# Infinidat/slimfastq

Hardware: AMD Instinct MI355X
Metric: MB/s FASTQ compressed (higher is better)
Workload: dtype u8/u32 integer; 1 GPU; synthetic 10M x 150 bp Illumina reads per GPU, full qlts+gens+recs, frozen tables (one chain per lane), -l 3; level=3, block_reads=1024, prior_step=-1, blocks_per_gpu=9766, tables=frozen, chains_per_gpu=253906, raw_bytes_per_gpu=3702038404, parallelism=1 GPU

## Files before the change

slimfastq_amd/csrc/api.cpp:

```cpp
#include <hip/hip_runtime.h>

#include <algorithm>
#include <cmath>
#include <cstdarg>
#include <cstdlib>
#include <cstdio>
#include <cstring>
#include <string>
#include <vector>
#include <chrono>
#include <functional>
#include <future>
#include <thread>
#include <atomic>
#include <mutex>
#include <condition_variable>

#include "kernels.h"

namespace {

struct HostTimes {
    bool on; std::chrono::steady_clock::time_point t0; std::vector<std::pair<const char*, double>> marks;
    HostTimes() : on(getenv("SFQ_HOST_TIMING") != nullptr), t0(std::chrono::steady_clock::now()) {}
// ... 51 lines not shown
    EE_HEAD_END,
    EE_M0_BEGIN, EE_M0_END, EE_M1_BEGIN, EE_M1_END, EE_M2_BEGIN, EE_M2_END, EE_M3_BEGIN, EE_M3_END,
    EE_PACK_BEGIN, EE_PACK_END,
    EE_FRAME_K_BEGIN,
    EE_TEXT_FORK,
    EE_QLT_CODE_BEGIN, EE_QLT_CODE_END,
    EE_GEN_CODE_BEGIN, EE_GEN_CODE_END,
    EE_REC_CODE_BEGIN,
    EE_NEVER_READ,
    EE_QLT_LIST_HOME,
    EE_QLT_ROWS_BUILT,
    EE_LINES_INDEXED,
    EE_FRAME_K_END,
    EE_REC_FREQS_HOME,
    EE_REC_CODE_END,
    EE_COUNT
};
enum {
    ED_BEGIN,
    ED_HEAD_END,
    ED_FORK,
    ED_QLT_END,
    ED_GEN_END,
    ED_REC_END,
    ED_END,
    ED_GEN_BEGIN,
    ED_OVER_FORK,
    ED_OVER_LINES_END,
    ED_LISTS_COPIED,
    ED_COUNT
// ... 9 lines not shown
    bool rec_copy_pending = false;
    bool rec_blob_pending = false;
    std::string err;
    u64 table_budget = 0;
    u64 dev_total = 0;
    u32 wave_slots = 8192;
    u32 epoch_base = 0;
    Tables tab;
    DevBuf chunk_base, scan_tmp, line_off, status, blocks, arena, blk_stream_off, stream_total,
           lens, blob_off, blob, in_stage, out_stage;
    DevBuf slen, qlen, pfg, pfq, soff, qoff, seq_stage, qual_stage, hdr_stage, hlen, hoff, hso, hsc, rsize, roff, d_first;
    DevBuf hist, rows66, ptmp, prior_w, prior_wovf, prior_ls, prior_lh, tickets;
    DevBuf gm_T, gm_slen, gm_boff, gm_soff, gm_scan, gm_stage, gm_tok, gm_csz, gm_idx;
    DevBuf qrows, qdec, qesc, qw, csz, coff, gcnt, grows, glog, gcost, gbins, gfill, hcnt, hfreq, rrows, rdec, rmap, rflags, rtok, excf, cflags;
    DevBuf chn_len, chn_off, chn_out;
    DevBuf pslot, plist;
    DevBuf segn, segoff, segrec;
    DevBuf oflags, okbytes, ofpos, okoff, ofilt, orecmap, olist, line_off_o, ono, opiece, otxt[3], osize_all, oroff_all, oroff_k, ocnt;
    u32 r_hot = 0, r_hot_dec = 0;
    bool blobs_from_encode = false;
    bool unsettled = false;
    bool counts_only = false; u32 sample_scale = 1;
    struct { const u8* ptr = nullptr; u64 nbytes = 0, nrec = 0, print = 0; bool marks = false, valid = false; } framed;
    struct { bool valid = false, rec = false; u32 q_rows = 0; } counts;
    void* pin = nullptr; size_t pin_cap = 0;
    void* pin2 = nullptr; size_t pin2_cap = 0;
    std::vector<u8> chain_blob;
    std::vector<u8> rec_prior_blob;
    std::vector<u8> chain_tmp;
    bool prior_on = false;
// ... 549 lines not shown
    const u32 ngen = gp.ngen = gen_bounds(nblocks, gp.bound);
    if (ngen < 3) return SFQ_OK;
    const u32* bound = gp.bound;
    int rc;
    gp.tb = gm_table_bits(ca.nbytes);
    const u64 br = ca.block_reads;
    gp.r2 = std::min<u64>(nrec, (u64)bound[2] * br);
    gp.cap = std::min<u64>(ca.nbytes, gp.r2 * ((u64)max_line + 1));
    if ((rc = reserve(ctx, ctx->gm_T, (size_t)8 << gp.tb))) return rc;
    if ((rc = reserve(ctx, ctx->gm_slen, (size_t)gp.r2 * 4 + 64))) return rc;
    if ((rc = reserve(ctx, ctx->gm_boff, ((size_t)gp.r2 + 1) * 8))) return rc;
    if ((rc = reserve(ctx, ctx->gm_soff, ((size_t)gp.r2 + 1) * 8))) return rc;
    if ((rc = reserve(ctx, ctx->gm_scan, ((size_t)nrec / 1024 + 4) * 8 + 65536))) return rc;
    if ((rc = reserve(ctx, ctx->gm_stage, (size_t)gp.cap + 64))) return rc;
    if ((rc = reserve(ctx, ctx->gcost, 64))) return rc;
    HIPC(hipMemsetAsync(ctx->gm_T.p, 0xFF, (size_t)8 << gp.tb, st));
    HIPC(hipMemsetAsync(ctx->gcost.p, 0, 64, st));
    if ((rc = gm_stage_upto(ctx, ca, gp.r2, 0, st))) return rc;
    gp.cg = ca;
    gp.cg.st_buf = (const u8*)ctx->gm_stage.p; gp.cg.st_bytes = gp.cap; gp.cg.st_off = (const u64*)ctx->gm_soff.p; gp.cg.st_len = (const u32*)ctx->gm_slen.p;
    auto recs = [&](u32 b0, u32 b1) { return (u64)(b1 - b0) * br; };
    launch_gm_insert(gp.cg, bound[0], bound[1], recs(bound[0], bound[1]), max_line, (u64*)ctx->gm_T.p, gp.tb, st);
    u16 costs[8];
    for (u32 lv = 0; lv < 4; lv++) {
        const u32 fo = lv == 0 ? 64u : lv == 1 ? 40u : lv == 2 ? 24u : 16u;
        costs[lv] = (u16)(12 * 1024 - log2fp_u32(4096u - 3u * fo)); costs[4 + lv] = (u16)(12 * 1024 - log2fp_u32(fo));
    }
    const u64 r1 = (u64)bound[1] * br;
    launch_gm_price(gp.cg, r1, gp.r2, (u64)gen_count_stride(recs(bound[1], bound[2])) * GEN_PRE, max_line, r1, (const u8*)ctx->gm_stage.p, gp.cap, (const u64*)ctx->gm_soff.p,
                    (const u32*)ctx->gm_slen.p, (const u64*)ctx->gm_T.p, gp.tb, costs, (u64*)ctx->gcost.p, st);
    HIPC(hipMemcpyAsync((u8*)ctx->pin + PIN_GEN_OFF, ctx->gcost.p, 16, hipMemcpyDeviceToHost, st));
    return SFQ_OK;
}
// ... 124 lines not shown
    ctx->table_budget = tot / 10 * 7;
    *out = ctx;
    return SFQ_OK;
}

void sfq_ctx_destroy(sfq_ctx* ctx) {
    if (!ctx) return;
    (void)hipSetDevice(ctx->dev);
    (void)hipStreamSynchronize(ctx->st);
    DevBuf* all[] = { &ctx->tab.q_slots, &ctx->tab.q_hdr, &ctx->tab.p_slots, &ctx->tab.p_hdr, &ctx->tab.g_tab,
        &ctx->chunk_base, &ctx->scan_tmp, &ctx->line_off, &ctx->status, &ctx->blocks, &ctx->arena,
        &ctx->blk_stream_off, &ctx->stream_total, &ctx->lens, &ctx->blob_off, &ctx->blob, &ctx->in_stage, &ctx->out_stage,
        &ctx->slen, &ctx->qlen, &ctx->pfg, &ctx->pfq, &ctx->soff, &ctx->qoff, &ctx->seq_stage, &ctx->qual_stage,
        &ctx->hdr_stage, &ctx->hlen, &ctx->hoff, &ctx->hso, &ctx->hsc, &ctx->rsize, &ctx->roff, &ctx->d_first,
        &ctx->hist, &ctx->rows66, &ctx->prior_w, &ctx->prior_wovf, &ctx->prior_ls, &ctx->prior_lh, &ctx->tickets,
        &ctx->hcnt, &ctx->hfreq, &ctx->rrows, &ctx->rdec, &ctx->rmap, &ctx->rflags, &ctx->rtok, &ctx->ptmp, &ctx->qrows, &ctx->qdec, &ctx->qesc, &ctx->qw, &ctx->csz, &ctx->coff, &ctx->gcnt, &ctx->grows, &ctx->glog, &ctx->gcost, &ctx->gbins, &ctx->gfill, &ctx->gm_T, &ctx->gm_slen, &ctx->gm_boff, &ctx->gm_soff, &ctx->gm_scan, &ctx->gm_stage, &ctx->gm_tok, &ctx->gm_csz, &ctx->gm_idx, &ctx->excf, &ctx->cflags, &ctx->segn, &ctx->segoff, &ctx->segrec, &ctx->pslot, &ctx->plist, &ctx->chn_len, &ctx->chn_off, &ctx->chn_out,
        &ctx->oflags, &ctx->okbytes, &ctx->ofpos, &ctx->okoff, &ctx->ofilt, &ctx->orecmap, &ctx->olist, &ctx->line_off_o, &ctx->ono, &ctx->opiece,
        &ctx->otxt[0], &ctx->otxt[1], &ctx->otxt[2], &ctx->osize_all, &ctx->oroff_all, &ctx->oroff_k, &ctx->ocnt,
        &ctx->crc_tab, &ctx->crc_tiles, &ctx->crc_grps, &ctx->crc_bounds, &ctx->crc_out, &ctx->stats_acc, &ctx->qmap_dev,
        &ctx->pair_work, &ctx->pair_in, &ctx->pair_out, &ctx->pick_out, &ctx->sel_out, &ctx->trim_out, &ctx->ovl_out, &ctx->mrg_out, &ctx->dd_out, &ctx->scr_out };
    for (DevBuf* b : all) release(*b);
    (void)sfq_dedup_set_destroy(ctx);
    (void)sfq_screen_set_destroy(ctx);
    if (ctx->pin) (void)hipHostFree(ctx->pin);
    if (ctx->pin2) (void)hipHostFree(ctx->pin2);
    if (ctx->crc_pin) (void)hipHostFree(ctx->crc_pin);
    for (auto& e : ctx->crc_ev) if (e) (void)hipEventDestroy(e);
    if (ctx->st_crc) (void)hipStreamDestroy(ctx->st_crc);
    if (ctx->stats_pin) (void)hipHostFree(ctx->stats_pin);
    if (ctx->qmap_pin) (void)hipHostFree(ctx->qmap_pin);
    if (ctx->pair_pin) (void)hipHostFree(ctx->pair_pin);
// ... 196 lines not shown
    const u32 block_reads = p.block_reads ? p.block_reads : (u32)std::min<u64>(nrec, 0xFFFFFFFFu);
    const u64 nblocks64 = (nrec + block_reads - 1) / block_reads;
    if (nblocks64 > (1u << 24)) return fail(ctx, SFQ_E_ARG, "too many blocks (%llu)", (unsigned long long)nblocks64);
    const u32 nblocks = (u32)nblocks64;
    const bool frozen = p.tables == SFQ_TABLES_FROZEN && p.block_reads != 0 && p.kernel == 0;
    int g_bits = p.gen_bits ? p.gen_bits : level_gen_bits(p.level);
    if (!p.gen_bits && p.block_reads) {
        const double bases = (frozen ? (double)nrec : (double)block_reads) * ((double)nbytes / (double)nrec) * 0.5;
        int cap = 12;
        while (cap < 26 && (double)(1u << cap) < bases) cap += 2;
        g_bits = std::min(g_bits, cap);
    }
    if (g_bits < 2 || g_bits > 26 ) return fail(ctx, SFQ_E_ARG, "gen_bits %d out of range", g_bits);
    if ((rc = reserve(ctx, ctx->blocks, (size_t)nblocks * sizeof(BlockDesc)))) return rc;
    launch_block_prepare(d_fastq, (const u64*)ctx->line_off.p, nrec, block_reads, (BlockDesc*)ctx->blocks.p, nblocks, nbytes, p.level, g_bits, st);
    const bool crc_pass = ctx->crc_on && !priors_only;
    if (crc_pass) {
        if ((rc = crc_reserve(ctx, d_fastq_in, 0, nbytes_in, nblocks))) return rc;
        HIPC(hipEventRecord(ctx->crc_ev[CRC_EV_FORK], st));
        HIPC(hipStreamWaitEvent(ctx->st_crc, ctx->crc_ev[CRC_EV_FORK], 0));
        launch_crc_block_bounds((const u64*)ctx->line_off.p, 4ull * block_reads, nblocks, nbytes_in, (u64*)ctx->crc_bounds.p, ctx->st_crc);
        if ((rc = crc_queue(ctx, d_fastq_in, nbytes_in, nblocks, ctx->st_crc))) return rc;
        HIPC(hipEventRecord(ctx->crc_ev[CRC_EV_DONE], ctx->st_crc));
    }
    const bool stats_pass = ctx->stats_on && !priors_only;
    if (stats_pass) {
        if ((rc = stats_ready(ctx))) return rc;
        HIPC(hipEventRecord(ctx->stats_ev[0], st));
        HIPC(hipStreamWaitEvent(ctx->st_stats, ctx->stats_ev[0], 0));
        HIPC(hipMemsetAsync(ctx->stats_acc.p, 0, (size_t)text_stats_acc_bytes(), ctx->st_stats));
// ... 17 lines not shown
            return fail(ctx, SFQ_E_ARG, "SFQ_PRIOR_COUNTS: no counts installed (sfq_set_prior_counts / sfq_count_priors come first; any other encode drops them)");
        if (ctx->counts.q_rows != q_rows) return fail(ctx, SFQ_E_ARG, "SFQ_PRIOR_COUNTS: the counts were installed for %u quality contexts, level %d has %u", ctx->counts.q_rows, p.level, q_rows);
        if (need_rec && !ctx->counts.rec) return fail(ctx, SFQ_E_ARG, "SFQ_PRIOR_COUNTS: the installed counts hold no header sample (they were counted for adaptive tables), frozen tables need one");
    }
    if (given && ctx->prior_blob.empty()) return fail(ctx, SFQ_E_ARG, "SFQ_PRIOR_GIVEN: no quality prior installed (sfq_set_qlt_prior)");
    if (given && frozen && (models & SFQ_M_REC) && ctx->rec_prior_blob.empty()) return fail(ctx, SFQ_E_ARG, "SFQ_PRIOR_GIVEN: no header prior installed (sfq_set_rec_prior)");
    if (!given) { ctx->prior_blob.clear(); ctx->rec_prior_blob.clear(); }
    ctx->rec_blob_pending = false; ctx->rec_copy_pending = false;
    ctx->chain_blob.clear();
    if (frozen && !prior_step) prior_step = SFQ_PRIOR_AUTO;
    u32 slots = 0;
    const u32 KR = 2;
    const u32 nblocks_r = (nblocks + KR - 1) / KR * KR;
    ModelArgs a;
    u32* tickets = nullptr;
    auto setup_tables = [&]() -> int {
        int rc;
        if ((rc = ensure_tables(ctx, nblocks_r, q_rows, (u32)g_bits, frozen ? (models & ~(SFQ_M_QLT | SFQ_M_GEN)) : models, &slots))) return rc;
        if (p.kernel == 0) {
            if (slots < KR) return fail(ctx, SFQ_E_NOMEM, "table budget %llu B holds %u block slot(s); the kernels need %u", (unsigned long long)ctx->table_budget, slots, KR);
            slots &= ~(KR - 1);
        }
        if ((rc = advance_epoch(ctx, nblocks))) return rc;
        fill_model_args(ctx, a, nblocks, p.level, (u32)g_bits, p.block_reads != 0);
        a.fq = d_fastq;
        a.rec_map = n_over ? (const u32*)ctx->orecmap.p : nullptr;
        if ((rc = reserve(ctx, ctx->tickets, 64))) return rc;
        HIPC(hipMemsetAsync(ctx->tickets.p, 0, 64, st));
        tickets = (u32*)ctx->tickets.p;
        return SFQ_OK;
    };
    const u32 order[4] = { SFQ_M_QLT, frozen ? SFQ_M_REC : SFQ_M_GEN, SFQ_M_USR, frozen ? SFQ_M_GEN : SFQ_M_REC };
    const int tslot[4] = { SFQ_T_QLT, frozen ? SFQ_T_REC : SFQ_T_GEN, SFQ_T_USR, frozen ? SFQ_T_GEN : SFQ_T_REC };
    hipStream_t mst[4] = { st, ctx->st_aux[0], ctx->st_aux[1], ctx->st_aux[2] };
    if (prior_step == SFQ_PRIOR_AUTO || (ctx->counts_only && prior_step == 0)) {
        const u64 per_rec = std::min<u64>(std::max<u64>(1, nbytes / nrec / 2), PRIOR_SYMBOLS);
        prior_step = (u32)std::min<u64>(std::max<u64>(1, nrec * per_rec / 24000000ull), 0x7FFFFFFFull);
        if (nbytes / nrec <= 4000) prior_step = (u32)std::max<u64>(prior_step, (nrec + 131071) / 131072);
    }
    if (ctx->counts_only && prior_step && prior_step < SFQ_PRIOR_COUNTS)
        prior_step = (u32)std::min<u64>((u64)prior_step * std::max<u32>(1u, ctx->sample_scale), 0x7FFFFFFFull);
    bool hist_launched = false;
    if (frozen && !given && !counted && prior_step && (models & SFQ_M_QLT)) {
// ... 9 lines not shown
    else HIPC(hipStreamSynchronize(st));
    const u32 h_status = h_status2[0], max_hdr = h_status2[1], max_line = h_status2[2], min_hdr = ~h_status2[4];
    if (h_status == (u32)(-SFQ_E_FORMAT)) return fail(ctx, SFQ_E_FORMAT, "fastq file: expecting '@' / '+' line prefixes (usrs.cpp:162-167)");
    if (h_status) return fail(ctx, -(int)h_status, "record over the line limits: headers up to 8190 bytes; base and quality lines up to 65534 in format 6 (-B 0; the reference would write oversize side streams, usrs.cpp:269-301, which this library does not), up to 1 Gi in the block format; or an empty base line");

    ChainArgs ca;
    memset(&ca, 0, sizeof ca);
    u32 nchains = 0, nsub = 0;
    GenPlan gplan; GmPlan gmplan;
    ChainGeoArgs ggeo; memset(&ggeo, 0, sizeof ggeo);
    const u32* gen_csz = nullptr;
    const bool flat_quads_req = getenv("SFQ_FLAT_QUADS") != nullptr;
    const bool gm = frozen && !exc_classic;
    u32 seg_len = 0;
    std::vector<u32> seg_blk;
    if (frozen) {
        u32 cr = p.chain_reads ? p.chain_reads : (u32)default_chain_reads(nrec, nbytes);
        if (p.chain_reads & SFQ_CHAIN_SEGMENT_FLAG) { seg_len = p.chain_reads & ~SFQ_CHAIN_SEGMENT_FLAG; cr = 1; if (!seg_len) return fail(ctx, SFQ_E_ARG, "SFQ_CHAIN_SEGMENT(0)"); }
        else if (!p.chain_reads && cr == 1 && nrec < 204800) {
            const u64 segs_want = SFQ_CHAINS_WANT - 8192 - std::min<u64>(nrec / 2, 100000);
            const u64 want = std::min<u64>(std::max<u64>(4096, nbytes / 2 / segs_want), 1u << 20);
            if (max_line > want) seg_len = (u32)want;
        }
        if (!p.chain_reads && !seg_len)
            while (cr < block_reads && (u64)nblocks * ((block_reads + cr - 1) / cr) > SFQ_CHAINS_WANT) cr++;
        ca.geo.chain_reads = (u32)std::min<u64>(std::min(cr, block_reads), nrec);
        ca.geo.cpb = (block_reads + ca.geo.chain_reads - 1) / ca.geo.chain_reads;
        if (!p.chain_reads) ca.geo.chain_reads = std::max<u32>(1u, (u32)((std::min<u64>(block_reads, nrec) + ca.geo.cpb - 1) / ca.geo.cpb));
        const u32 last_nrec = (u32)(nrec - (u64)(nblocks - 1) * block_reads);
        const u64 nc = (u64)(nblocks - 1) * ca.geo.cpb + (last_nrec + ca.geo.chain_reads - 1) / ca.geo.chain_reads;
// ... 15 lines not shown
            for (u32 b = 0; b < nblocks; b++) seg_blk[b] = (u32)(h_off[std::min<u64>((u64)(b + 1) * block_reads, nrec)] - h_off[(u64)b * block_reads]);
            if ((rc = reserve(ctx, ctx->segrec, (size_t)nchains * 4 + 16))) return rc;
            launch_seg_fill((const u64*)ctx->segoff.p, nrec, (u32*)ctx->segrec.p, st);
            ca.seg_len = seg_len; ca.seg_off = (const u64*)ctx->segoff.p; ca.seg_rec = (const u32*)ctx->segrec.p;
        }
        {
            const u32 cpb_want = std::max<u32>(1u, 61440u / nblocks);
            const u32 rfloor = nbytes / nrec > 4000 ? 16u : 128u;
            const u32 rcr0 = std::max<u32>(rfloor, (block_reads + cpb_want - 1) / cpb_want);
            const u32 rcr = (u32)std::min<u64>(std::min<u32>(std::max<u32>(rcr0, ca.geo.chain_reads), block_reads), nrec);
            ca.rgeo.chain_reads = rcr;
            ca.rgeo.cpb = (block_reads + rcr - 1) / rcr;
            nsub = ca.rgeo.nchains = (u32)((u64)(nblocks - 1) * ca.rgeo.cpb + (last_nrec + rcr - 1) / rcr);
        }
        if ((rc = reserve(ctx, ctx->csz, ((size_t)nchains * 2 + (size_t)nsub * 2) * 4))) return rc;
        HIPC(hipMemsetAsync(ctx->csz.p, 0, ((size_t)nchains * 2 + (size_t)nsub * 2) * 4, st));
        ggeo = ca.geo;
        if (gm && !seg_len) {
            const u64 per_rec = std::max<u64>(1, nbytes / std::max<u64>(1, nrec));
            const u64 gwant = std::max<u64>((GM_CHAIN_FLOOR + per_rec - 1) / per_rec, (nrec + GM_CHAIN_WANT - 1) / GM_CHAIN_WANT);
            const u32 gfloor = (u32)std::min<u64>(gwant, ca.geo.chain_reads);
            ggeo.cpb = (block_reads + gfloor - 1) / gfloor;
            ggeo.chain_reads = std::max<u32>(1u, (u32)((std::min<u64>(block_reads, nrec) + ggeo.cpb - 1) / ggeo.cpb));
            ggeo.cpb = (block_reads + ggeo.chain_reads - 1) / ggeo.chain_reads;
            const u64 ngc = (u64)(nblocks - 1) * ggeo.cpb + (last_nrec + ggeo.chain_reads - 1) / ggeo.chain_reads;
            if (ngc > 0x7FFFFFFFull || ggeo.chain_reads >= ca.geo.chain_reads) ggeo = ca.geo;
            else {
                ggeo.nchains = (u32)ngc;
                if ((rc = reserve(ctx, ctx->gm_csz, (size_t)ggeo.nchains * 4))) return rc;
                HIPC(hipMemsetAsync(ctx->gm_csz.p, 0, (size_t)ggeo.nchains * 4, st));
            }
        }
        if ((rc = reserve_pinned(ctx, PIN_BYTES + (size_t)q_rows * 66 * 4))) return rc;
        if ((rc = setup_tables())) return rc;
        HIPC(hipEventRecord(ctx->ev[EE_TEXT_FORK], st));
        if (!priors_only) {
            for (int m = 1; m < 4; m++) { HIPC(hipStreamWaitEvent(mst[m], ctx->ev[EE_TEXT_FORK], 0)); HIPC(hipEventRecord(ev_model_begin(ctx, m), mst[m])); }
            a.batch0 = 0; a.nbatch = std::min(slots, nblocks_r);
            ca.m = a;
            if (models & SFQ_M_REC) { if ((rc = rec_prior_begin(ctx, a, nrec, given, counted, mst[1], max_hdr))) return rc; }
            if (models & SFQ_M_GEN) {
                if (gm) { if ((rc = gm_begin(ctx, ca, nblocks, nrec, max_line, mst[3], gmplan))) return rc; }
                else if ((rc = gen_tables_begin(ctx, ca, nblocks, (u32)g_bits, max_line, mst[3], gplan))) return rc;
            }
        } else if (models & SFQ_M_REC) {
            HIPC(hipStreamWaitEvent(mst[1], ctx->ev[EE_TEXT_FORK], 0));
            if ((rc = rec_prior_begin(ctx, a, nrec, given, counted, mst[1], max_hdr))) return rc;
        }
    }
    u32* h_rows66 = nullptr;
    if (given && (models & SFQ_M_QLT)) {
        if ((rc = ensure_prior_buffers(ctx, q_rows))) return rc;
        if (!hist_cleared) HIPC(hipMemsetAsync(ctx->hist.p, 0, (size_t)q_rows * 64 * 4, st));
        if ((rc = upload_prior(ctx, q_rows, st, !frozen))) return rc;
        HIPC(hipEventRecord(ctx->ev[EE_HEAD_END], st));
        ctx->prior_on = true;
    } else if (prior_step && (models & SFQ_M_QLT)) {
        if ((rc = ensure_prior_buffers(ctx, q_rows))) return rc;
// ... 35 lines not shown
            launch_qlt_frozen_rows((const u32*)ctx->rows66.p, q_rows, (u32*)ctx->qrows.p, nullptr, st);
            ca.qrows = (const u32*)ctx->qrows.p; ca.qesc = (const u32*)ctx->qesc.p;
            ca.q_hot = 0; ca.q_rows = q_rows;
            const u32 want_hot = (p.lds_rows == SFQ_LDS_ROWS_NONE || given || !prior_step) ? 0u : p.lds_rows ? std::min<u32>(p.lds_rows, 1024u)
                                 : nchains >= 150000u ? 800u : 0u;
            if (want_hot) {
                const size_t img_bytes = (size_t)q_rows / 4 + (size_t)want_hot * 100 + 64;
                if ((rc = reserve(ctx, ctx->qw, img_bytes + (size_t)q_rows * 4 + 256))) return rc;
                u8* img = (u8*)ctx->qw.p; u32* info = (u32*)(img + ((img_bytes + 15) & ~(size_t)15)); u32* ctot = info + 16;
                launch_hot_rows((const u32*)ctx->hist.p, (const u32*)ctx->rows66.p, (const u32*)ctx->qrows.p, q_rows, want_hot, ctot, img, info, st);
                ca.q_hot = want_hot; ca.qh_img = img; ca.qh_info = info;
            }
            HIPC(hipEventRecord(ctx->ev[EE_HEAD_END], st));
        }
    }
    if (!frozen) { if ((rc = setup_tables())) return rc; }
    if (priors_only) {
        if (ctx->prior_on && !given) {
            if ((rc = qlt_prior_blob_now(ctx, h_rows66, q_rows, st))) return rc;
        }
        if (frozen && (models & SFQ_M_REC)) { if ((rc = rec_prior_finish(ctx, given, mst[1]))) return rc; if ((rc = rec_prior_copy_back(ctx, mst[1]))) return rc; if ((rc = rec_prior_blob_now(ctx))) return rc; }
        HIPC(hipStreamSynchronize(mst[1]));
        HIPC(hipStreamSynchronize(st));
        ctx->prior_on = false;
        res->n_records = nrec; res->n_blocks = nblocks;
        return SFQ_OK;
    }
    u32 gen_on = 0;
    const bool exc_rice = frozen && !exc_classic;
    if (frozen) {
        a.batch0 = 0; a.nbatch = std::min(slots, nblocks_r);
// ... 80 lines not shown
                }
            }
        }
        if (order[m] == SFQ_M_USR && n_over) {
            const u64 ooff[3] = { arena_main, arena_main + over_cap, arena_main + 2 * over_cap };
            const u32 ocap[3] = { (u32)over_cap, (u32)over_cap, (u32)over_cap };
            launch_over_encode_w(a, d_file, (const u64*)ctx->line_off_o.p, (const u32*)ctx->olist.p, n_over, ooff, ocap, mst[m]);
        }
        HIPC(hipEventRecord(ev_model_end(ctx, m), mst[m]));
        if (m) HIPC(hipStreamWaitEvent(st, ev_model_end(ctx, m), 0));
    }
    }
    ht.mark("chains queued");
    HIPC(hipEventRecord(ctx->ev[EE_PACK_BEGIN], st));

    if ((rc = reserve(ctx, ctx->blk_stream_off, (size_t)nblocks * SFQ_NSTREAMS * 8))) return rc;
    if ((rc = reserve(ctx, ctx->stream_total, 2 * SFQ_NSTREAMS * 8 + 64))) return rc;
    u32 chain_streams = 0;
    if (frozen) {
        ca.m = a;
        if (models & SFQ_M_QLT) { launch_chain_block_sizes(ca, ca.geo, SFQ_S_QLT, (const u32*)ctx->csz.p, nullptr, st); chain_streams |= 1u << SFQ_S_QLT; }
        if (models & SFQ_M_GEN) { launch_chain_block_sizes(ca, ggeo, SFQ_S_GEN, gen_csz, nullptr, st); chain_streams |= 1u << SFQ_S_GEN; }
        if (models & SFQ_M_REC) {
            const u32* rs = (const u32*)ctx->csz.p + 2 * (size_t)nchains;
            launch_chain_block_sizes(ca, ca.rgeo, SFQ_S_REC, rs, rs + nsub, st); chain_streams |= 1u << SFQ_S_REC;
        }
    }
    launch_block_stream_offsets((BlockDesc*)ctx->blocks.p, nblocks, (u64*)ctx->blk_stream_off.p, (u64*)ctx->stream_total.p, st);
    if ((rc = reserve(ctx, ctx->lens, (size_t)nblocks * 4))) return rc;
    if ((rc = reserve(ctx, ctx->blob_off, ((size_t)nblocks + 1) * 8))) return rc;
    const u64 blob_cap = std::min<u64>(nbytes, (u64)nblocks * SFQ_MAX_ID_LLEN);
    if ((rc = reserve(ctx, ctx->blob, blob_cap))) return rc;
    launch_first_hdr_lens((const BlockDesc*)ctx->blocks.p, nblocks, (u32*)ctx->lens.p, st);
    launch_scan_u32((const u32*)ctx->lens.p, (u64*)ctx->blob_off.p, nblocks, (u64*)ctx->scan_tmp.p, st);
    launch_gather_first_hdrs((const BlockDesc*)ctx->blocks.p, nblocks, d_fastq, (const u64*)ctx->blob_off.p, (u8*)ctx->blob.p, blob_cap, st);
    const size_t p2_hb = 128, p2_off = p2_hb + (((size_t)nblocks * sizeof(BlockDesc) + 63) & ~(size_t)63);
    const size_t p2_csz = p2_off + ((((size_t)nblocks + 1) * 8 + 63) & ~(size_t)63);
    const u32 ngc = frozen ? ggeo.nchains : 0;
    const bool gsplit = frozen && ngc != nchains;
    const size_t n_sizes = (size_t)nchains + ngc + (size_t)nsub * 2;
    const u32* d_sizes = (const u32*)ctx->csz.p;
    if (gsplit) {
        if ((rc = reserve(ctx, ctx->gm_idx, n_sizes * 4 + 64))) return rc;
        u32* di = (u32*)ctx->gm_idx.p;
        HIPC(hipMemcpyAsync(di, ctx->csz.p, (size_t)nchains * 4, hipMemcpyDeviceToDevice, st));
        HIPC(hipMemcpyAsync(di + nchains, ctx->gm_csz.p, (size_t)ngc * 4, hipMemcpyDeviceToDevice, st));
        HIPC(hipMemcpyAsync(di + nchains + ngc, (const u32*)ctx->csz.p + 2 * (size_t)nchains, (size_t)nsub * 2 * 4, hipMemcpyDeviceToDevice, st));
        d_sizes = di;
    }
    const size_t p2_end = p2_csz + n_sizes * 4 + 64;
    if ((rc = reserve_pinned_buf(ctx, ctx->pin2, ctx->pin2_cap, p2_end))) return rc;
    u64* totals = (u64*)ctx->pin2;
    HIPC(hipMemcpyAsync(totals, ctx->stream_total.p, SFQ_NSTREAMS * 8, hipMemcpyDeviceToHost, st));
    auto pack_prior_now = [&]() -> int {
        if (ctx->prior_on && !given && h_rows66) {
            if ((rc = qlt_prior_blob_now(ctx, h_rows66, q_rows, mst[2]))) return rc;
            h_rows66 = nullptr;
        }
        return rec_prior_blob_now(ctx);
    };
    BlockDesc* hb = (BlockDesc*)((u8*)ctx->pin2 + p2_hb);
    u64* hboff = (u64*)((u8*)ctx->pin2 + p2_off);
    u32* h_csz = (u32*)((u8*)ctx->pin2 + p2_csz);
    const bool rec_chains = (chain_streams >> SFQ_S_REC) & 1;
    const u32 chn_n = frozen ? nchains + ngc + (rec_chains ? nsub * 2 : 0u) : 0u;
    const size_t chn_eager = std::min<size_t>((size_t)chn_n * 5, n_sizes * 4 + 64 - 16);
    u32* d_gate = (u32*)((u64*)ctx->stream_total.p + 2 * SFQ_NSTREAMS);
    const u64 blob_guess = std::min<u64>(blob_cap, (u64)nblocks * 256);
    launch_stream_gate((const BlockDesc*)ctx->blocks.p, nblocks, (const u64*)ctx->stream_total.p, out_cap, (u64*)ctx->stream_total.p + SFQ_NSTREAMS, d_gate, st);
    launch_compact((const BlockDesc*)ctx->blocks.p, nblocks, (const u8*)ctx->arena.p, (const u64*)ctx->blk_stream_off.p,
                   (const u64*)ctx->stream_total.p + SFQ_NSTREAMS, d_out, chain_streams, st, d_gate);
    if (frozen) {
        if (chain_streams & (1u << SFQ_S_QLT))
            launch_compact_chains(ca, ca.geo, SFQ_S_QLT, 2, 1, (const u32*)ctx->csz.p, (const u64*)ctx->blk_stream_off.p, (const u64*)ctx->stream_total.p + SFQ_NSTREAMS, d_out, st, d_gate);
        if (chain_streams & (1u << SFQ_S_GEN))
            launch_compact_chains(ca, ggeo, SFQ_S_GEN, 3, 4, gen_csz, (const u64*)ctx->blk_stream_off.p, (const u64*)ctx->stream_total.p + SFQ_NSTREAMS, d_out, st, d_gate);
        if (chain_streams & (1u << SFQ_S_REC))
            launch_compact_chains(ca, ca.rgeo, SFQ_S_REC, 3, 2, (const u32*)ctx->csz.p + 2 * (size_t)nchains, (const u64*)ctx->blk_stream_off.p, (const u64*)ctx->stream_total.p + SFQ_NSTREAMS, d_out, st, d_gate);
        {
            const u32 b1 = nchains, b2 = nchains + ngc, b3 = rec_chains ? nchains + ngc + nsub : chn_n;
            if ((rc = reserve(ctx, ctx->chn_len, (size_t)chn_n * 4 + 16))) return rc;
            if ((rc = reserve(ctx, ctx->chn_off, ((size_t)chn_n + 4) * 8))) return rc;
            if ((rc = reserve(ctx, ctx->chn_out, (size_t)chn_n * 5 + 64))) return rc;
            if ((rc = reserve(ctx, ctx->scan_tmp, ((size_t)chn_n / 1024 + 4) * 8 + 65536))) return rc;
            u64* d_info = (u64*)ctx->chn_off.p + chn_n + 1;
            launch_chain_index_bytes(d_sizes, chn_n, b1, b2 > chn_n ? chn_n : b2, b3, (u32*)ctx->chn_len.p, (u64*)ctx->chn_off.p, (u64*)ctx->scan_tmp.p,
                                     (u8*)ctx->chn_out.p, d_info, st);
            HIPC(hipMemcpyAsync(h_csz, d_info, 16, hipMemcpyDeviceToHost, st));
            if (chn_eager) HIPC(hipMemcpyAsync((u8*)h_csz + 16, ctx->chn_out.p, chn_eager, hipMemcpyDeviceToHost, st));
        }
    }
    HIPC(hipEventRecord(ctx->ev[EE_PACK_END], st));
    if ((rc = pack_prior_now())) return rc;
    ctx->first_hdrs.resize((size_t)blob_guess);
    if (blob_guess) HIPC(hipMemcpyAsync(ctx->first_hdrs.data(), ctx->blob.p, (size_t)blob_guess, hipMemcpyDeviceToHost, st));
    HIPC(hipMemcpyAsync(hb, ctx->blocks.p, (size_t)nblocks * sizeof(BlockDesc), hipMemcpyDeviceToHost, st));
    HIPC(hipMemcpyAsync(hboff, ctx->blob_off.p, ((size_t)nblocks + 1) * 8, hipMemcpyDeviceToHost, st));
    ht.mark("packing queued");
    if ((rc = pack_prior_now())) return rc;
    ht.mark("priors packed");
    HIPC(hipStreamSynchronize(st));
    ht.mark("device through");
    u64 bases[SFQ_NSTREAMS], run = 0;
    for (int s = 0; s < SFQ_NSTREAMS; s++) { bases[s] = run; run += totals[s]; res->stream_bytes[s] = totals[s]; res->stream_offset[s] = bases[s]; }
    res->total_bytes = run;
    int worst = 0;
    for (u32 b = 0; b < nblocks; b++) if (hb[b].status) worst = std::max<int>(worst, (int)hb[b].status);
    if (worst) return fail(ctx, -worst, "block kernel reported error %d (%s)", -worst,
                           -worst == SFQ_E_OVERFLOW ? "stream arena too small" : -worst == SFQ_E_GENCHAR ? "unexpected genome char / switched N byte" :
                           -worst == SFQ_E_UNSUPPORTED ? "a '+' line that is neither empty nor its record's header: the block format refuses what it could not give back (usrs.cpp:236-239)" : "see status codes");
    ht.mark("  statuses looked at");
    if (run > out_cap) return fail(ctx, SFQ_E_OVERFLOW, "output needs %llu bytes, caller gave %llu", (unsigned long long)run, (unsigned long long)out_cap);
    if (hboff[nblocks] > blob_cap) return fail(ctx, SFQ_E_OVERFLOW, "first-header blob overflow");
    if (hboff[nblocks] > blob_guess) {
        ctx->first_hdrs.resize((size_t)hboff[nblocks]);
        HIPC(hipMemcpyAsync(ctx->first_hdrs.data() + blob_guess, (const u8*)ctx->blob.p + blob_guess, (size_t)(hboff[nblocks] - blob_guess), hipMemcpyDeviceToHost, st));
        HIPC(hipStreamSynchronize(st));
    } else ctx->first_hdrs.resize((size_t)hboff[nblocks]);

    ht.mark("  first headers home");
    ctx->prior_on = false;
    ctx->chain_blob.clear();
    if (frozen) {
        std::vector<u8>& o = ctx->chain_tmp;
        const size_t o_need = ((size_t)nchains + ngc + (size_t)nsub * 2 + (seg_len ? nblocks : 0)) * 5 + 64;
        if (o.size() < o_need) o.resize(o_need);
        u8* w = o.data();
        auto put = [&w](u32 v) { while (v >= 0x80) { *w++ = (u8)(v | 0x80); v >>= 7; } *w++ = (u8)v; };
// ... 2475 lines not shown
```

Before: 369,200 MB/s.

## Move first-header gather, size clears and chain indexing onto side streams

In the frozen gen-match path, the first-header length/scan/gather and its host copies now run on an auxiliary model stream during the head phase, into pinned memory. The memsets of the chain-size arrays move onto the model streams that write them. The chain index build and its copies run on a side stream alongside compaction instead of serially on the main stream. The goal is to take small serial kernels and copies off the critical path, at the cost of more event dependencies and a pinned staging buffer sized up front.

```diff
diff --git a/slimfastq_amd/csrc/api.cpp b/slimfastq_amd/csrc/api.cpp
--- a/slimfastq_amd/csrc/api.cpp
+++ b/slimfastq_amd/csrc/api.cpp
@@ -89,6 +89,10 @@
     EE_FRAME_K_END,
     EE_REC_FREQS_HOME,
     EE_REC_CODE_END,
+    EE_BLOCKS_READY,
+    EE_GEN_SIZES_CLEAR,
+    EE_SIZES_SET,
+    EE_SIDE_END,
     EE_COUNT
 };
 enum {
@@ -128,6 +132,7 @@
     DevBuf gm_T, gm_slen, gm_boff, gm_soff, gm_scan, gm_stage, gm_tok, gm_csz, gm_idx;
     DevBuf qrows, qdec, qesc, qw, csz, coff, gcnt, grows, glog, gcost, gbins, gfill, hcnt, hfreq, rrows, rdec, rmap, rflags, rtok, excf, cflags;
     DevBuf chn_len, chn_off, chn_out;
+    DevBuf side_scan;
     DevBuf pslot, plist;
     DevBuf segn, segoff, segrec;
     DevBuf oflags, okbytes, ofpos, okoff, ofilt, orecmap, olist, line_off_o, ono, opiece, otxt[3], osize_all, oroff_all, oroff_k, ocnt;
@@ -707,9 +712,9 @@
     if ((rc = reserve(ctx, ctx->gm_scan, ((size_t)nrec / 1024 + 4) * 8 + 65536))) return rc;
     if ((rc = reserve(ctx, ctx->gm_stage, (size_t)gp.cap + 64))) return rc;
     if ((rc = reserve(ctx, ctx->gcost, 64))) return rc;
+    if ((rc = gm_stage_upto(ctx, ca, gp.r2, 0, st))) return rc;
     HIPC(hipMemsetAsync(ctx->gm_T.p, 0xFF, (size_t)8 << gp.tb, st));
     HIPC(hipMemsetAsync(ctx->gcost.p, 0, 64, st));
-    if ((rc = gm_stage_upto(ctx, ca, gp.r2, 0, st))) return rc;
     gp.cg = ca;
     gp.cg.st_buf = (const u8*)ctx->gm_stage.p; gp.cg.st_bytes = gp.cap; gp.cg.st_off = (const u64*)ctx->gm_soff.p; gp.cg.st_len = (const u32*)ctx->gm_slen.p;
     auto recs = [&](u32 b0, u32 b1) { return (u64)(b1 - b0) * br; };
@@ -864,7 +869,7 @@
         &ctx->slen, &ctx->qlen, &ctx->pfg, &ctx->pfq, &ctx->soff, &ctx->qoff, &ctx->seq_stage, &ctx->qual_stage,
         &ctx->hdr_stage, &ctx->hlen, &ctx->hoff, &ctx->hso, &ctx->hsc, &ctx->rsize, &ctx->roff, &ctx->d_first,
         &ctx->hist, &ctx->rows66, &ctx->prior_w, &ctx->prior_wovf, &ctx->prior_ls, &ctx->prior_lh, &ctx->tickets,
-        &ctx->hcnt, &ctx->hfreq, &ctx->rrows, &ctx->rdec, &ctx->rmap, &ctx->rflags, &ctx->rtok, &ctx->ptmp, &ctx->qrows, &ctx->qdec, &ctx->qesc, &ctx->qw, &ctx->csz, &ctx->coff, &ctx->gcnt, &ctx->grows, &ctx->glog, &ctx->gcost, &ctx->gbins, &ctx->gfill, &ctx->gm_T, &ctx->gm_slen, &ctx->gm_boff, &ctx->gm_soff, &ctx->gm_scan, &ctx->gm_stage, &ctx->gm_tok, &ctx->gm_csz, &ctx->gm_idx, &ctx->excf, &ctx->cflags, &ctx->segn, &ctx->segoff, &ctx->segrec, &ctx->pslot, &ctx->plist, &ctx->chn_len, &ctx->chn_off, &ctx->chn_out,
+        &ctx->hcnt, &ctx->hfreq, &ctx->rrows, &ctx->rdec, &ctx->rmap, &ctx->rflags, &ctx->rtok, &ctx->ptmp, &ctx->qrows, &ctx->qdec, &ctx->qesc, &ctx->qw, &ctx->csz, &ctx->coff, &ctx->gcnt, &ctx->grows, &ctx->glog, &ctx->gcost, &ctx->gbins, &ctx->gfill, &ctx->gm_T, &ctx->gm_slen, &ctx->gm_boff, &ctx->gm_soff, &ctx->gm_scan, &ctx->gm_stage, &ctx->gm_tok, &ctx->gm_csz, &ctx->gm_idx, &ctx->excf, &ctx->cflags, &ctx->segn, &ctx->segoff, &ctx->segrec, &ctx->pslot, &ctx->plist, &ctx->chn_len, &ctx->chn_off, &ctx->chn_out, &ctx->side_scan,
         &ctx->oflags, &ctx->okbytes, &ctx->ofpos, &ctx->okoff, &ctx->ofilt, &ctx->orecmap, &ctx->olist, &ctx->line_off_o, &ctx->ono, &ctx->opiece,
         &ctx->otxt[0], &ctx->otxt[1], &ctx->otxt[2], &ctx->osize_all, &ctx->oroff_all, &ctx->oroff_k, &ctx->ocnt,
         &ctx->crc_tab, &ctx->crc_tiles, &ctx->crc_grps, &ctx->crc_bounds, &ctx->crc_out, &ctx->stats_acc, &ctx->qmap_dev,
@@ -1091,6 +1096,7 @@
     if (g_bits < 2 || g_bits > 26 ) return fail(ctx, SFQ_E_ARG, "gen_bits %d out of range", g_bits);
     if ((rc = reserve(ctx, ctx->blocks, (size_t)nblocks * sizeof(BlockDesc)))) return rc;
     launch_block_prepare(d_fastq, (const u64*)ctx->line_off.p, nrec, block_reads, (BlockDesc*)ctx->blocks.p, nblocks, nbytes, p.level, g_bits, st);
+    HIPC(hipEventRecord(ctx->ev[EE_BLOCKS_READY], st));
     const bool crc_pass = ctx->crc_on && !priors_only;
     if (crc_pass) {
         if ((rc = crc_reserve(ctx, d_fastq_in, 0, nbytes_in, nblocks))) return rc;
@@ -1138,7 +1144,7 @@
     const u32 nblocks_r = (nblocks + KR - 1) / KR * KR;
     ModelArgs a;
     u32* tickets = nullptr;
-    auto setup_tables = [&]() -> int {
+    auto setup_tables = [&](hipStream_t tst) -> int {
         int rc;
         if ((rc = ensure_tables(ctx, nblocks_r, q_rows, (u32)g_bits, frozen ? (models & ~(SFQ_M_QLT | SFQ_M_GEN)) : models, &slots))) return rc;
         if (p.kernel == 0) {
@@ -1150,7 +1156,7 @@
         a.fq = d_fastq;
         a.rec_map = n_over ? (const u32*)ctx->orecmap.p : nullptr;
         if ((rc = reserve(ctx, ctx->tickets, 64))) return rc;
-        HIPC(hipMemsetAsync(ctx->tickets.p, 0, 64, st));
+        HIPC(hipMemsetAsync(ctx->tickets.p, 0, 64, tst));
         tickets = (u32*)ctx->tickets.p;
         return SFQ_OK;
     };
@@ -1190,6 +1196,22 @@
     const bool gm = frozen && !exc_classic;
     u32 seg_len = 0;
     std::vector<u32> seg_blk;
+    bool gm_split = false;
+    const u64 blob_cap = std::min<u64>(nbytes, (u64)nblocks * SFQ_MAX_ID_LLEN);
+    const u64 blob_guess = std::min<u64>(blob_cap, (u64)nblocks * 256);
+    auto first_hdrs_queue = [&](hipStream_t fst, u64* tmp) {
+        launch_first_hdr_lens((const BlockDesc*)ctx->blocks.p, nblocks, (u32*)ctx->lens.p, fst);
+        launch_scan_u32((const u32*)ctx->lens.p, (u64*)ctx->blob_off.p, nblocks, tmp, fst);
+        launch_gather_first_hdrs((const BlockDesc*)ctx->blocks.p, nblocks, d_fastq, (const u64*)ctx->blob_off.p, (u8*)ctx->blob.p, blob_cap, fst);
+    };
+    const size_t p2_hb = 128, p2_off = p2_hb + (((size_t)nblocks * sizeof(BlockDesc) + 63) & ~(size_t)63);
+    const size_t p2_blob = p2_off + ((((size_t)nblocks + 1) * 8 + 63) & ~(size_t)63);
+    size_t p2_csz = p2_blob, p2_sizes = 0;
+    auto pin2_reserve = [&](size_t n_sizes, bool with_blob) -> int {
+        p2_csz = p2_blob + (with_blob ? (((size_t)blob_guess + 63) & ~(size_t)63) : 0);
+        p2_sizes = n_sizes;
+        return reserve_pinned_buf(ctx, ctx->pin2, ctx->pin2_cap, p2_csz + n_sizes * 4 + 64);
+    };
     if (frozen) {
         u32 cr = p.chain_reads ? p.chain_reads : (u32)default_chain_reads(nrec, nbytes);
         if (p.chain_reads & SFQ_CHAIN_SEGMENT_FLAG) { seg_len = p.chain_reads & ~SFQ_CHAIN_SEGMENT_FLAG; cr = 1; if (!seg_len) return fail(ctx, SFQ_E_ARG, "SFQ_CHAIN_SEGMENT(0)"); }
@@ -1235,7 +1257,7 @@
             nsub = ca.rgeo.nchains = (u32)((u64)(nblocks - 1) * ca.rgeo.cpb + (last_nrec + rcr - 1) / rcr);
         }
         if ((rc = reserve(ctx, ctx->csz, ((size_t)nchains * 2 + (size_t)nsub * 2) * 4))) return rc;
-        HIPC(hipMemsetAsync(ctx->csz.p, 0, ((size_t)nchains * 2 + (size_t)nsub * 2) * 4, st));
+        if (!gm) HIPC(hipMemsetAsync(ctx->csz.p, 0, ((size_t)nchains * 2 + (size_t)nsub * 2) * 4, st));
         ggeo = ca.geo;
         if (gm && !seg_len) {
             const u64 per_rec = std::max<u64>(1, nbytes / std::max<u64>(1, nrec));
@@ -1249,20 +1271,42 @@
             else {
                 ggeo.nchains = (u32)ngc;
                 if ((rc = reserve(ctx, ctx->gm_csz, (size_t)ggeo.nchains * 4))) return rc;
-                HIPC(hipMemsetAsync(ctx->gm_csz.p, 0, (size_t)ggeo.nchains * 4, st));
+                gm_split = true;
             }
         }
         if ((rc = reserve_pinned(ctx, PIN_BYTES + (size_t)q_rows * 66 * 4))) return rc;
-        if ((rc = setup_tables())) return rc;
+        if (gm && !priors_only) {
+            const size_t sizes_most = (size_t)nchains + std::max(nchains, ggeo.nchains) + (size_t)nsub * 2;
+            if ((rc = reserve(ctx, ctx->lens, (size_t)nblocks * 4))) return rc;
+            if ((rc = reserve(ctx, ctx->blob_off, ((size_t)nblocks + 1) * 8))) return rc;
+            if ((rc = reserve(ctx, ctx->blob, blob_cap))) return rc;
+            if ((rc = reserve(ctx, ctx->side_scan, (sizes_most / 1024 + 4) * 8 + 65536))) return rc;
+            if ((rc = pin2_reserve(sizes_most, true))) return rc;
+        }
+        if ((rc = setup_tables(gm ? mst[2] : st))) return rc;
         HIPC(hipEventRecord(ctx->ev[EE_TEXT_FORK], st));
+        if (gm) HIPC(hipMemsetAsync(ctx->csz.p, 0, (size_t)nchains * 4, st));
         if (!priors_only) {
-            for (int m = 1; m < 4; m++) { HIPC(hipStreamWaitEvent(mst[m], ctx->ev[EE_TEXT_FORK], 0)); HIPC(hipEventRecord(ev_model_begin(ctx, m), mst[m])); }
+            for (int m = 1; m < 4; m++) {
+                HIPC(hipStreamWaitEvent(mst[m], ctx->ev[gm && m == 3 ? EE_BLOCKS_READY : EE_TEXT_FORK], 0));
+                HIPC(hipEventRecord(ev_model_begin(ctx, m), mst[m]));
+            }
             a.batch0 = 0; a.nbatch = std::min(slots, nblocks_r);
             ca.m = a;
+            if (gm && (models & SFQ_M_GEN)) { if ((rc = gm_begin(ctx, ca, nblocks, nrec, max_line, mst[3], gmplan))) return rc; }
+            if (gm) {
+                HIPC(hipMemsetAsync((u32*)ctx->csz.p + nchains, 0, (size_t)nchains * 4, mst[2]));
+                if (gm_split) HIPC(hipMemsetAsync(ctx->gm_csz.p, 0, (size_t)ggeo.nchains * 4, mst[2]));
+                HIPC(hipEventRecord(ctx->ev[EE_GEN_SIZES_CLEAR], mst[2]));
+                HIPC(hipStreamWaitEvent(mst[3], ctx->ev[EE_GEN_SIZES_CLEAR], 0));
+                HIPC(hipMemsetAsync((u32*)ctx->csz.p + 2 * (size_t)nchains, 0, (size_t)nsub * 2 * 4, mst[1]));
+            }
             if (models & SFQ_M_REC) { if ((rc = rec_prior_begin(ctx, a, nrec, given, counted, mst[1], max_hdr))) return rc; }
-            if (models & SFQ_M_GEN) {
-                if (gm) { if ((rc = gm_begin(ctx, ca, nblocks, nrec, max_line, mst[3], gmplan))) return rc; }
-                else if ((rc = gen_tables_begin(ctx, ca, nblocks, (u32)g_bits, max_line, mst[3], gplan))) return rc;
+            if (!gm && (models & SFQ_M_GEN)) { if ((rc = gen_tables_begin(ctx, ca, nblocks, (u32)g_bits, max_line, mst[3], gplan))) return rc; }
+            if (gm) {
+                first_hdrs_queue(mst[2], (u64*)ctx->side_scan.p);
+                HIPC(hipMemcpyAsync((u8*)ctx->pin2 + p2_off, ctx->blob_off.p, ((size_t)nblocks + 1) * 8, hipMemcpyDeviceToHost, mst[2]));
+                if (blob_guess) HIPC(hipMemcpyAsync((u8*)ctx->pin2 + p2_blob, ctx->blob.p, (size_t)blob_guess, hipMemcpyDeviceToHost, mst[2]));
             }
         } else if (models & SFQ_M_REC) {
             HIPC(hipStreamWaitEvent(mst[1], ctx->ev[EE_TEXT_FORK], 0));
@@ -1328,7 +1372,7 @@
             HIPC(hipEventRecord(ctx->ev[EE_HEAD_END], st));
         }
     }
-    if (!frozen) { if ((rc = setup_tables())) return rc; }
+    if (!frozen) { if ((rc = setup_tables(st))) return rc; }
     if (priors_only) {
         if (ctx->prior_on && !given) {
             if ((rc = qlt_prior_blob_now(ctx, h_rows66, q_rows, st))) return rc;
@@ -1439,6 +1483,9 @@
     ht.mark("chains queued");
     HIPC(hipEventRecord(ctx->ev[EE_PACK_BEGIN], st));
 
+    const bool side = gm;
+    hipStream_t sst = side ? mst[2] : st;
+    if (side) HIPC(hipStreamWaitEvent(sst, ctx->ev[EE_PACK_BEGIN], 0));
     if ((rc = reserve(ctx, ctx->blk_stream_off, (size_t)nblocks * SFQ_NSTREAMS * 8))) return rc;
     if ((rc = reserve(ctx, ctx->stream_total, 2 * SFQ_NSTREAMS * 8 + 64))) return rc;
     u32 chain_streams = 0;
@@ -1452,15 +1499,13 @@
         }
     }
     launch_block_stream_offsets((BlockDesc*)ctx->blocks.p, nblocks, (u64*)ctx->blk_stream_off.p, (u64*)ctx->stream_total.p, st);
-    if ((rc = reserve(ctx, ctx->lens, (size_t)nblocks * 4))) return rc;
-    if ((rc = reserve(ctx, ctx->blob_off, ((size_t)nblocks + 1) * 8))) return rc;
-    const u64 blob_cap = std::min<u64>(nbytes, (u64)nblocks * SFQ_MAX_ID_LLEN);
-    if ((rc = reserve(ctx, ctx->blob, blob_cap))) return rc;
-    launch_first_hdr_lens((const BlockDesc*)ctx->blocks.p, nblocks, (u32*)ctx->lens.p, st);
-    launch_scan_u32((const u32*)ctx->lens.p, (u64*)ctx->blob_off.p, nblocks, (u64*)ctx->scan_tmp.p, st);
-    launch_gather_first_hdrs((const BlockDesc*)ctx->blocks.p, nblocks, d_fastq, (const u64*)ctx->blob_off.p, (u8*)ctx->blob.p, blob_cap, st);
-    const size_t p2_hb = 128, p2_off = p2_hb + (((size_t)nblocks * sizeof(BlockDesc) + 63) & ~(size_t)63);
-    const size_t p2_csz = p2_off + ((((size_t)nblocks + 1) * 8 + 63) & ~(size_t)63);
+    if (side) HIPC(hipEventRecord(ctx->ev[EE_SIZES_SET], st));
+    else {
+        if ((rc = reserve(ctx, ctx->lens, (size_t)nblocks * 4))) return rc;
+        if ((rc = reserve(ctx, ctx->blob_off, ((size_t)nblocks + 1) * 8))) return rc;
+        if ((rc = reserve(ctx, ctx->blob, blob_cap))) return rc;
+        first_hdrs_queue(st, (u64*)ctx->scan_tmp.p);
+    }
     const u32 ngc = frozen ? ggeo.nchains : 0;
     const bool gsplit = frozen && ngc != nchains;
     const size_t n_sizes = (size_t)nchains + ngc + (size_t)nsub * 2;
@@ -1468,13 +1513,13 @@
     if (gsplit) {
         if ((rc = reserve(ctx, ctx->gm_idx, n_sizes * 4 + 64))) return rc;
         u32* di = (u32*)ctx->gm_idx.p;
-        HIPC(hipMemcpyAsync(di, ctx->csz.p, (size_t)nchains * 4, hipMemcpyDeviceToDevice, st));
-        HIPC(hipMemcpyAsync(di + nchains, ctx->gm_csz.p, (size_t)ngc * 4, hipMemcpyDeviceToDevice, st));
-        HIPC(hipMemcpyAsync(di + nchains + ngc, (const u32*)ctx->csz.p + 2 * (size_t)nchains, (size_t)nsub * 2 * 4, hipMemcpyDeviceToDevice, st));
+        HIPC(hipMemcpyAsync(di, ctx->csz.p, (size_t)nchains * 4, hipMemcpyDeviceToDevice, sst));
+        HIPC(hipMemcpyAsync(di + nchains, ctx->gm_csz.p, (size_t)ngc * 4, hipMemcpyDeviceToDevice, sst));
+        HIPC(hipMemcpyAsync(di + nchains + ngc, (const u32*)ctx->csz.p + 2 * (size_t)nchains, (size_t)nsub * 2 * 4, hipMemcpyDeviceToDevice, sst));
         d_sizes = di;
     }
-    const size_t p2_end = p2_csz + n_sizes * 4 + 64;
-    if ((rc = reserve_pinned_buf(ctx, ctx->pin2, ctx->pin2_cap, p2_end))) return rc;
+    if (!side) { if ((rc = pin2_reserve(n_sizes, false))) return rc; }
+    else if (n_sizes > p2_sizes) return fail(ctx, SFQ_E_HIP, "chain sizes: %zu where the head made room for %zu", n_sizes, p2_sizes);
     u64* totals = (u64*)ctx->pin2;
     HIPC(hipMemcpyAsync(totals, ctx->stream_total.p, SFQ_NSTREAMS * 8, hipMemcpyDeviceToHost, st));
     auto pack_prior_now = [&]() -> int {
@@ -1491,7 +1536,6 @@
     const u32 chn_n = frozen ? nchains + ngc + (rec_chains ? nsub * 2 : 0u) : 0u;
     const size_t chn_eager = std::min<size_t>((size_t)chn_n * 5, n_sizes * 4 + 64 - 16);
     u32* d_gate = (u32*)((u64*)ctx->stream_total.p + 2 * SFQ_NSTREAMS);
-    const u64 blob_guess = std::min<u64>(blob_cap, (u64)nblocks * 256);
     launch_stream_gate((const BlockDesc*)ctx->blocks.p, nblocks, (const u64*)ctx->stream_total.p, out_cap, (u64*)ctx->stream_total.p + SFQ_NSTREAMS, d_gate, st);
     launch_compact((const BlockDesc*)ctx->blocks.p, nblocks, (const u8*)ctx->arena.p, (const u64*)ctx->blk_stream_off.p,
                    (const u64*)ctx->stream_total.p + SFQ_NSTREAMS, d_out, chain_streams, st, d_gate);
@@ -1507,20 +1551,29 @@
             if ((rc = reserve(ctx, ctx->chn_len, (size_t)chn_n * 4 + 16))) return rc;
             if ((rc = reserve(ctx, ctx->chn_off, ((size_t)chn_n + 4) * 8))) return rc;
             if ((rc = reserve(ctx, ctx->chn_out, (size_t)chn_n * 5 + 64))) return rc;
-            if ((rc = reserve(ctx, ctx->scan_tmp, ((size_t)chn_n / 1024 + 4) * 8 + 65536))) return rc;
+            DevBuf& chn_scan = side ? ctx->side_scan : ctx->scan_tmp;
+            if ((rc = reserve(ctx, chn_scan, ((size_t)chn_n / 1024 + 4) * 8 + 65536))) return rc;
             u64* d_info = (u64*)ctx->chn_off.p + chn_n + 1;
-            launch_chain_index_bytes(d_sizes, chn_n, b1, b2 > chn_n ? chn_n : b2, b3, (u32*)ctx->chn_len.p, (u64*)ctx->chn_off.p, (u64*)ctx->scan_tmp.p,
-                                     (u8*)ctx->chn_out.p, d_info, st);
-            HIPC(hipMemcpyAsync(h_csz, d_info, 16, hipMemcpyDeviceToHost, st));
-            if (chn_eager) HIPC(hipMemcpyAsync((u8*)h_csz + 16, ctx->chn_out.p, chn_eager, hipMemcpyDeviceToHost, st));
-        }
+            launch_chain_index_bytes(d_sizes, chn_n, b1, b2 > chn_n ? chn_n : b2, b3, (u32*)ctx->chn_len.p, (u64*)ctx->chn_off.p, (u64*)chn_scan.p,
+                                     (u8*)ctx->chn_out.p, d_info, sst);
+            HIPC(hipMemcpyAsync(h_csz, d_info, 16, hipMemcpyDeviceToHost, sst));
+            if (chn_eager) HIPC(hipMemcpyAsync((u8*)h_csz + 16, ctx->chn_out.p, chn_eager, hipMemcpyDeviceToHost, sst));
+        }
+    }
+    if (side) {
+        HIPC(hipStreamWaitEvent(sst, ctx->ev[EE_SIZES_SET], 0));
+        HIPC(hipMemcpyAsync(hb, ctx->blocks.p, (size_t)nblocks * sizeof(BlockDesc), hipMemcpyDeviceToHost, sst));
+        HIPC(hipEventRecord(ctx->ev[EE_SIDE_END], sst));
+        HIPC(hipStreamWaitEvent(st, ctx->ev[EE_SIDE_END], 0));
     }
     HIPC(hipEventRecord(ctx->ev[EE_PACK_END], st));
-    if ((rc = pack_prior_now())) return rc;
-    ctx->first_hdrs.resize((size_t)blob_guess);
-    if (blob_guess) HIPC(hipMemcpyAsync(ctx->first_hdrs.data(), ctx->blob.p, (size_t)blob_guess, hipMemcpyDeviceToHost, st));
-    HIPC(hipMemcpyAsync(hb, ctx->blocks.p, (size_t)nblocks * sizeof(BlockDesc), hipMemcpyDeviceToHost, st));
-    HIPC(hipMemcpyAsync(hboff, ctx->blob_off.p, ((size_t)nblocks + 1) * 8, hipMemcpyDeviceToHost, st));
+    if (!side) {
+        if ((rc = pack_prior_now())) return rc;
+        ctx->first_hdrs.resize((size_t)blob_guess);
+        if (blob_guess) HIPC(hipMemcpyAsync(ctx->first_hdrs.data(), ctx->blob.p, (size_t)blob_guess, hipMemcpyDeviceToHost, st));
+        HIPC(hipMemcpyAsync(hb, ctx->blocks.p, (size_t)nblocks * sizeof(BlockDesc), hipMemcpyDeviceToHost, st));
+        HIPC(hipMemcpyAsync(hboff, ctx->blob_off.p, ((size_t)nblocks + 1) * 8, hipMemcpyDeviceToHost, st));
+    }
     ht.mark("packing queued");
     if ((rc = pack_prior_now())) return rc;
     ht.mark("priors packed");
@@ -1537,6 +1590,11 @@
     ht.mark("  statuses looked at");
     if (run > out_cap) return fail(ctx, SFQ_E_OVERFLOW, "output needs %llu bytes, caller gave %llu", (unsigned long long)run, (unsigned long long)out_cap);
     if (hboff[nblocks] > blob_cap) return fail(ctx, SFQ_E_OVERFLOW, "first-header blob overflow");
+    if (side) {
+        const size_t got = (size_t)std::min<u64>(hboff[nblocks], blob_guess);
+        ctx->first_hdrs.resize(got);
+        if (got) memcpy(ctx->first_hdrs.data(), (const u8*)ctx->pin2 + p2_blob, got);
+    }
     if (hboff[nblocks] > blob_guess) {
         ctx->first_hdrs.resize((size_t)hboff[nblocks]);
         HIPC(hipMemcpyAsync(ctx->first_hdrs.data() + blob_guess, (const u8*)ctx->blob.p + blob_guess, (size_t)(hboff[nblocks] - blob_guess), hipMemcpyDeviceToHost, st));
```

New measurement: 379,100 MB/s, median of 6. 2.7% higher.
